# lambdaclass/ethrex

Measured on NVIDIA B200. Metric: bn254_g1_msm_points_per_sec, higher is better.
Workload: dtype u32x8 Montgomery (254-bit modular integer)

## Files before the change

### ethrex_b200/csrc/common.cuh

```cuda
#pragma once
#include <cuda_runtime.h>
#include <nvtx3/nvToolsExt.h>
#include <cstdint>
#include <cstdio>
#include <map>
#include <string>
#include <vector>

#include "../../include/b200zk.h"
#include "curve.cuh"
#include "bls381.cuh"

namespace b200zk {

template <> struct CurveB<Fp381> {
  static B2_D Fp381 b() { Fp381 four = Fp381::zero(); four.v[0] = 4; return Fp381::to_mont(four); }
};

struct DevBuf {
  void* p = nullptr;
  size_t cap = 0;
};

struct TwiddleSet {
  void* d = nullptr;
  size_t bytes = 0;
  uint32_t gen[8] = {0, 0, 0, 0, 0, 0, 0, 0};
  uint32_t root[8] = {0, 0, 0, 0, 0, 0, 0, 0};
  cudaEvent_t ready = nullptr;
};

struct SortSlot {
  DevBuf hist, offsets, cursor, run_off, tsum, digits, idx, key, ctab, cnt2;
  cudaEvent_t sorted = nullptr, released = nullptr;
};

struct BasesEntry {
  void* d = nullptr;
  size_t n = 0;
  bool g2 = false;
  bool bls = false;
  uint32_t table_c = 0;
};

}

struct b200zk_ctx {
  int device = 0;
  int sm_count = 148;
  cudaStream_t stream = nullptr;
  std::string last_error;
  uint64_t launches = 0;
  uint32_t msm_window = 0;
  uint32_t msm_chunks = 0;
  cudaStream_t stream_sort = nullptr;
  cudaEvent_t ev_in = nullptr;
  cudaEvent_t ev_up[64] = {};
  b200zk::SortSlot slot[2];
  b200zk::DevBuf ws_totals, ws_bitpart;
  b200zk::DevBuf ws_key, ws_ctab, ws_cnt2;
  b200zk::DevBuf ws_g16[4];
  b200zk::DevBuf ws_zinv;
  uint32_t zinv_log_n = 0xffffffffu;
  bool attr_sort = false, attr_acc = false, attr_ntt512 = false, attr_ntt256 = false;
  int msm_pair_rounds = -1;
  bool profiling = false;
  float phase_ms[6] = {0, 0, 0, 0, 0, 0};
  cudaEvent_t ev[8] = {};
  b200zk::DevBuf ws_hist, ws_offsets, ws_cursor, ws_blocksums, ws_idx, ws_buckets, ws_chunkS, ws_chunkV, ws_result,
      ws_points, ws_scalars, ws_ntt, ws_misc, ws_out, ws_segoff, ws_segbucket, ws_digits, ws_q0, ws_q1, ws_prefix, ws_info, ws_pairoff0, ws_pairoff1;
  uint32_t ntt_root[8] = {0x725b19f0u, 0x9bd61b6eu, 0x41112ed4u, 0x402d111eu, 0x8ef62abcu, 0x00e0a7ebu, 0xa58a7e85u, 0x2a3c09f0u};
  uint64_t ntt_root_id = 0;
  std::map<uint64_t, b200zk::TwiddleSet> twiddles;
  std::map<uint64_t, b200zk::BasesEntry> bases;
  uint64_t next_handle = 1;
  uint8_t* h_pinned = nullptr;
};

namespace b200zk {

inline int fail(b200zk_ctx* ctx, int status, const char* what, cudaError_t e = cudaSuccess) {
  if (ctx) {
    ctx->last_error = what;
    if (e != cudaSuccess) { ctx->last_error += ": "; ctx->last_error += cudaGetErrorString(e); }
  }
  return status;
}

#define B2_CUDA(ctx, expr)                                                      \
  do {                                                                          \
    cudaError_t _e = (expr);                                                    \
    if (_e != cudaSuccess) return b200zk::fail(ctx, _e == cudaErrorMemoryAllocation ? B200ZK_ERR_OOM : B200ZK_ERR_CUDA, #expr, _e); \
  } while (0)

#define B2_TRY(expr)                        \
  do {                                      \
    int _s = (expr);                        \
    if (_s > B200ZK_OK_INFINITY) return _s; \
  } while (0)

inline int ensure(b200zk_ctx* ctx, DevBuf& b, size_t bytes) {
  if (bytes <= b.cap) return B200ZK_OK;
  B2_CUDA(ctx, cudaDeviceSynchronize());
  if (b.p) { cudaFree(b.p); b.p = nullptr; b.cap = 0; }
  size_t want = bytes + bytes / 8;
  cudaError_t e = cudaMalloc(&b.p, want);
  if (e != cudaSuccess) { cudaGetLastError(); want = bytes; e = cudaMalloc(&b.p, want); }
  if (e != cudaSuccess) { cudaGetLastError(); b.p = nullptr; return fail(ctx, B200ZK_ERR_OOM, "cudaMalloc workspace", e); }
  b.cap = want;
  return B200ZK_OK;
}

struct DeviceGuard {
  int prev = -1;
  bool switched = false;
  explicit DeviceGuard(const b200zk_ctx* ctx) {
    if (!ctx) return;
    if (cudaGetDevice(&prev) != cudaSuccess) { cudaGetLastError(); prev = -1; }
    if (prev != ctx->device) { switched = cudaSetDevice(ctx->device) == cudaSuccess; if (!switched) cudaGetLastError(); }
  }
  ~DeviceGuard() { if (switched && prev >= 0) cudaSetDevice(prev); }
  DeviceGuard(const DeviceGuard&) = delete;
  DeviceGuard& operator=(const DeviceGuard&) = delete;
};

struct NvtxRange {
  explicit NvtxRange(const char* name) { nvtxRangePushA(name); }
  ~NvtxRange() { nvtxRangePop(); }
  NvtxRange(const NvtxRange&) = delete;
  NvtxRange& operator=(const NvtxRange&) = delete;
};

inline cudaStream_t pick_stream(b200zk_ctx* ctx, void* stream) { return stream ? (cudaStream_t)stream : ctx->stream; }

#define B2_LAUNCH(ctx, kernel, grid, block, smem, st, ...)                                   \
  do {                                                                                       \
    kernel<<<(grid), (block), (smem), (st)>>>(__VA_ARGS__);                                  \
    (ctx)->launches++;                                                                       \
    cudaError_t _e = cudaGetLastError();                                                     \
    if (_e != cudaSuccess) return b200zk::fail(ctx, B200ZK_ERR_CUDA, "launch " #kernel, _e); \
  } while (0)

template <class F> B2_D F load_fe(const void* base, size_t index) {
  const uint4* p = reinterpret_cast<const uint4*>(base) + 2 * index;
  uint4 lo = p[0], hi = p[1];
  F r;
  r.v[0] = lo.x; r.v[1] = lo.y; r.v[2] = lo.z; r.v[3] = lo.w;
// ... 91 lines not shown
```

### ethrex_b200/csrc/field.cuh

```cuda
#pragma once
#include <cstdint>

#define B2_HD __host__ __device__ __forceinline__
#define B2_D __device__ __forceinline__

namespace b200zk {

struct FqCfg {
  static B2_HD constexpr uint32_t mod(int i) {
    constexpr uint32_t m[8] = {0xd87cfd47u, 0x3c208c16u, 0x6871ca8du, 0x97816a91u, 0x8181585du, 0xb85045b6u, 0xe131a029u, 0x30644e72u};
    return m[i];
  }
  static B2_HD constexpr uint32_t r1(int i) {
    constexpr uint32_t m[8] = {0xc58f0d9du, 0xd35d438du, 0xf5c70b3du, 0x0a78eb28u, 0x7879462cu, 0x666ea36fu, 0x9a07df2fu, 0x0e0a77c1u};
    return m[i];
  }
  static B2_HD constexpr uint32_t r2(int i) {
    constexpr uint32_t m[8] = {0x538afa89u, 0xf32cfc5bu, 0xd44501fbu, 0xb5e71911u, 0x0a417ff6u, 0x47ab1effu, 0xcab8351fu, 0x06d89f71u};
    return m[i];
  }
  static constexpr uint32_t INV = 0xe4866389u;
};

struct FrCfg {
// ... 67 lines not shown
      : "r"(a2), "r"(a4), "r"(a6), "r"(b));
}
B2_D void mad_even_z2(uint32_t* x, uint32_t& top, uint32_t a4, uint32_t a6, uint32_t b) {
  asm("mad.lo.cc.u32  %0, %5, %7, %0;\n\t"
      "madc.hi.cc.u32 %1, %5, %7, %1;\n\t"
      "madc.lo.cc.u32 %2, %6, %7, %2;\n\t"
      "madc.hi.cc.u32 %3, %6, %7, %3;\n\t"
      "addc.u32       %4, %4, 0;"
      : "+r"(x[4]), "+r"(x[5]), "+r"(x[6]), "+r"(x[7]), "+r"(top)
      : "r"(a4), "r"(a6), "r"(b));
}
B2_D void mad_even_z3(uint32_t* x, uint32_t& top, uint32_t a6, uint32_t b) {
  asm("mad.lo.cc.u32  %0, %3, %4, %0;\n\t"
      "madc.hi.cc.u32 %1, %3, %4, %1;\n\t"
      "addc.u32       %2, %2, 0;"
      : "+r"(x[6]), "+r"(x[7]), "+r"(top)
      : "r"(a6), "r"(b));
}
B2_D void shift_mad_odd_z1(uint32_t* e, uint32_t& x0, uint32_t a3, uint32_t a5, uint32_t a7, uint32_t b) {
  asm("add.cc.u32     %8, %8, %1;\n\t"
      "addc.cc.u32    %0, %2, 0;\n\t"
      "addc.cc.u32    %1, %3, 0;\n\t"
      "madc.lo.cc.u32 %2, %9, %12, %4;\n\t"
      "madc.hi.cc.u32 %3, %9, %12, %5;\n\t"
      "madc.lo.cc.u32 %4, %10, %12, %6;\n\t"
      "madc.hi.cc.u32 %5, %10, %12, %7;\n\t"
      "madc.lo.cc.u32 %6, %11, %12, 0;\n\t"
      "madc.hi.u32    %7, %11, %12, 0;"
      : "+r"(e[0]), "+r"(e[1]), "+r"(e[2]), "+r"(e[3]), "+r"(e[4]), "+r"(e[5]), "+r"(e[6]), "+r"(e[7]), "+r"(x0)
      : "r"(a3), "r"(a5), "r"(a7), "r"(b));
}
B2_D void shift_mad_odd_z2(uint32_t* e, uint32_t& x0, uint32_t a5, uint32_t a7, uint32_t b) {
  asm("add.cc.u32     %8, %8, %1;\n\t"
      "addc.cc.u32    %0, %2, 0;\n\t"
      "addc.cc.u32    %1, %3, 0;\n\t"
      "addc.cc.u32    %2, %4, 0;\n\t"
      "addc.cc.u32    %3, %5, 0;\n\t"
      "madc.lo.cc.u32 %4, %9, %11, %6;\n\t"
      "madc.hi.cc.u32 %5, %9, %11, %7;\n\t"
      "madc.lo.cc.u32 %6, %10, %11, 0;\n\t"
      "madc.hi.u32    %7, %10, %11, 0;"
      : "+r"(e[0]), "+r"(e[1]), "+r"(e[2]), "+r"(e[3]), "+r"(e[4]), "+r"(e[5]), "+r"(e[6]), "+r"(e[7]), "+r"(x0)
      : "r"(a5), "r"(a7), "r"(b));
}
B2_D void shift_mad_odd_z3(uint32_t* e, uint32_t& x0, uint32_t a7, uint32_t b) {
  asm("add.cc.u32     %8, %8, %1;\n\t"
      "addc.cc.u32    %0, %2, 0;\n\t"
      "addc.cc.u32    %1, %3, 0;\n\t"
      "addc.cc.u32    %2, %4, 0;\n\t"
      "addc.cc.u32    %3, %5, 0;\n\t"
      "addc.cc.u32    %4, %6, 0;\n\t"
      "addc.cc.u32    %5, %7, 0;\n\t"
      "madc.lo.cc.u32 %6, %9, %10, 0;\n\t"
      "madc.hi.u32    %7, %9, %10, 0;"
      : "+r"(e[0]), "+r"(e[1]), "+r"(e[2]), "+r"(e[3]), "+r"(e[4]), "+r"(e[5]), "+r"(e[6]), "+r"(e[7]), "+r"(x0)
      : "r"(a7), "r"(b));
}

B2_D void mul_even(uint32_t* x, uint32_t a0, uint32_t a2, uint32_t a4, uint32_t a6, uint32_t b) {
  asm("mul.lo.u32 %0, %8,  %12;\n\t mul.hi.u32 %1, %8,  %12;\n\t"
      "mul.lo.u32 %2, %9,  %12;\n\t mul.hi.u32 %3, %9,  %12;\n\t"
      "mul.lo.u32 %4, %10, %12;\n\t mul.hi.u32 %5, %10, %12;\n\t"
      "mul.lo.u32 %6, %11, %12;\n\t mul.hi.u32 %7, %11, %12;"
      : "=r"(x[0]), "=r"(x[1]), "=r"(x[2]), "=r"(x[3]), "=r"(x[4]), "=r"(x[5]), "=r"(x[6]), "=r"(x[7])
      : "r"(a0), "r"(a2), "r"(a4), "r"(a6), "r"(b));
}

B2_D void add8(uint32_t* r, const uint32_t* a, const uint32_t* b) {
  asm("add.cc.u32  %0, %8,  %16;\n\t addc.cc.u32 %1, %9,  %17;\n\t addc.cc.u32 %2, %10, %18;\n\t addc.cc.u32 %3, %11, %19;\n\t"
      "addc.cc.u32 %4, %12, %20;\n\t addc.cc.u32 %5, %13, %21;\n\t addc.cc.u32 %6, %14, %22;\n\t addc.u32    %7, %15, %23;"
      : "=r"(r[0]), "=r"(r[1]), "=r"(r[2]), "=r"(r[3]), "=r"(r[4]), "=r"(r[5]), "=r"(r[6]), "=r"(r[7])
      : "r"(a[0]), "r"(a[1]), "r"(a[2]), "r"(a[3]), "r"(a[4]), "r"(a[5]), "r"(a[6]), "r"(a[7]),
        "r"(b[0]), "r"(b[1]), "r"(b[2]), "r"(b[3]), "r"(b[4]), "r"(b[5]), "r"(b[6]), "r"(b[7]));
}
B2_D uint32_t sub8(uint32_t* r, const uint32_t* a, const uint32_t* b) {
  uint32_t borrow;
  asm("sub.cc.u32  %0, %9,  %17;\n\t subc.cc.u32 %1, %10, %18;\n\t subc.cc.u32 %2, %11, %19;\n\t subc.cc.u32 %3, %12, %20;\n\t"
      "subc.cc.u32 %4, %13, %21;\n\t subc.cc.u32 %5, %14, %22;\n\t subc.cc.u32 %6, %15, %23;\n\t subc.cc.u32 %7, %16, %24;\n\t"
      "subc.u32    %8, 0, 0;"
      : "=r"(r[0]), "=r"(r[1]), "=r"(r[2]), "=r"(r[3]), "=r"(r[4]), "=r"(r[5]), "=r"(r[6]), "=r"(r[7]), "=r"(borrow)
      : "r"(a[0]), "r"(a[1]), "r"(a[2]), "r"(a[3]), "r"(a[4]), "r"(a[5]), "r"(a[6]), "r"(a[7]),
        "r"(b[0]), "r"(b[1]), "r"(b[2]), "r"(b[3]), "r"(b[4]), "r"(b[5]), "r"(b[6]), "r"(b[7]));
  return borrow;
}

}

template <class Cfg>
struct Fe {
  uint32_t v[8];

  static B2_HD Fe zero() { Fe r; for (int i = 0; i < 8; ++i) r.v[i] = 0; return r; }
  static B2_HD Fe one() { Fe r; for (int i = 0; i < 8; ++i) r.v[i] = Cfg::r1(i); return r; }
  static B2_HD Fe rsquared() { Fe r; for (int i = 0; i < 8; ++i) r.v[i] = Cfg::r2(i); return r; }
  static B2_HD Fe modulus() { Fe r; for (int i = 0; i < 8; ++i) r.v[i] = Cfg::mod(i); return r; }

  B2_HD bool is_zero() const {
    uint32_t o = 0;
#pragma unroll
    for (int i = 0; i < 8; ++i) o |= v[i];
    return o == 0;
  }
  B2_HD bool operator==(const Fe& b) const {
    uint32_t o = 0;
#pragma unroll
    for (int i = 0; i < 8; ++i) o |= v[i] ^ b.v[i];
    return o == 0;
  }
  B2_HD bool operator!=(const Fe& b) const { return !(*this == b); }

  static B2_D Fe reduce_once(const Fe& a) {
    Fe m = modulus(), t;
    uint32_t borrow = detail::sub8(t.v, a.v, m.v);
    Fe r;
#pragma unroll
    for (int i = 0; i < 8; ++i) r.v[i] = borrow ? a.v[i] : t.v[i];
    return r;
  }
  static B2_D Fe add(const Fe& a, const Fe& b) {
    Fe s; detail::add8(s.v, a.v, b.v);
    return reduce_once(s);
  }
  static B2_D Fe sub(const Fe& a, const Fe& b) {
    Fe d; uint32_t borrow = detail::sub8(d.v, a.v, b.v);
    Fe m;
#pragma unroll
    for (int i = 0; i < 8; ++i) m.v[i] = Cfg::mod(i) & borrow;
    Fe r; detail::add8(r.v, d.v, m.v);
    return r;
  }
  static B2_D Fe dbl(const Fe& a) { return add(a, a); }
  static B2_D Fe neg(const Fe& a) {
    Fe m = modulus(), r; detail::sub8(r.v, m.v, a.v);
    uint32_t nz = a.is_zero() ? 0u : 0xffffffffu;
#pragma unroll
    for (int i = 0; i < 8; ++i) r.v[i] &= nz;
    return r;
  }

  static B2_D Fe mul(const Fe& a, const Fe& b) {
    uint32_t ev[8], od[8];
    uint32_t m;
    detail::mul_even(ev, a.v[0], a.v[2], a.v[4], a.v[6], b.v[0]);
    detail::mul_even(od, a.v[1], a.v[3], a.v[5], a.v[7], b.v[0]);
    m = ev[0] * Cfg::INV;
    detail::mad_odd(od, Cfg::mod(1), Cfg::mod(3), Cfg::mod(5), Cfg::mod(7), m);
    detail::mad_even(ev, od[7], Cfg::mod(0), Cfg::mod(2), Cfg::mod(4), Cfg::mod(6), m);
#pragma unroll
    for (int i = 1; i < 8; i += 2) {
      detail::shift_mad_odd(ev, od[0], a.v[1], a.v[3], a.v[5], a.v[7], b.v[i]);
      detail::mad_even(od, ev[7], a.v[0], a.v[2], a.v[4], a.v[6], b.v[i]);
      m = od[0] * Cfg::INV;
      detail::mad_odd(ev, Cfg::mod(1), Cfg::mod(3), Cfg::mod(5), Cfg::mod(7), m);
      detail::mad_even(od, ev[7], Cfg::mod(0), Cfg::mod(2), Cfg::mod(4), Cfg::mod(6), m);
      if (i + 1 < 8) {
        detail::shift_mad_odd(od, ev[0], a.v[1], a.v[3], a.v[5], a.v[7], b.v[i + 1]);
        detail::mad_even(ev, od[7], a.v[0], a.v[2], a.v[4], a.v[6], b.v[i + 1]);
        m = ev[0] * Cfg::INV;
        detail::mad_odd(od, Cfg::mod(1), Cfg::mod(3), Cfg::mod(5), Cfg::mod(7), m);
        detail::mad_even(ev, od[7], Cfg::mod(0), Cfg::mod(2), Cfg::mod(4), Cfg::mod(6), m);
      }
    }
    Fe r;
    asm("add.cc.u32  %0, %8,  %16;\n\t addc.cc.u32 %1, %9,  %17;\n\t addc.cc.u32 %2, %10, %18;\n\t addc.cc.u32 %3, %11, %19;\n\t"
        "addc.cc.u32 %4, %12, %20;\n\t addc.cc.u32 %5, %13, %21;\n\t addc.cc.u32 %6, %14, %22;\n\t addc.u32    %7, %15, 0;"
        : "=r"(r.v[0]), "=r"(r.v[1]), "=r"(r.v[2]), "=r"(r.v[3]), "=r"(r.v[4]), "=r"(r.v[5]), "=r"(r.v[6]), "=r"(r.v[7])
// ... 80 lines not shown
        detail::mad_even(ev, od[7], c.v[0], c.v[2], c.v[4], c.v[6], d.v[i + 1]);
        m = ev[0] * Cfg::INV;
        detail::mad_odd(od, Cfg::mod(1), Cfg::mod(3), Cfg::mod(5), Cfg::mod(7), m);
        detail::mad_even(ev, od[7], Cfg::mod(0), Cfg::mod(2), Cfg::mod(4), Cfg::mod(6), m);
      }
    }
    Fe r;
    asm("add.cc.u32  %0, %8,  %16;\n\t addc.cc.u32 %1, %9,  %17;\n\t addc.cc.u32 %2, %10, %18;\n\t addc.cc.u32 %3, %11, %19;\n\t"
        "addc.cc.u32 %4, %12, %20;\n\t addc.cc.u32 %5, %13, %21;\n\t addc.cc.u32 %6, %14, %22;\n\t addc.u32    %7, %15, 0;"
        : "=r"(r.v[0]), "=r"(r.v[1]), "=r"(r.v[2]), "=r"(r.v[3]), "=r"(r.v[4]), "=r"(r.v[5]), "=r"(r.v[6]), "=r"(r.v[7])
        : "r"(ev[0]), "r"(ev[1]), "r"(ev[2]), "r"(ev[3]), "r"(ev[4]), "r"(ev[5]), "r"(ev[6]), "r"(ev[7]),
          "r"(od[1]), "r"(od[2]), "r"(od[3]), "r"(od[4]), "r"(od[5]), "r"(od[6]), "r"(od[7]));
    return reduce_once(r);
  }
  static B2_D Fe mul4_add(const Fe& a, const Fe& b, const Fe& c, const Fe& d, const Fe& e, const Fe& f, const Fe& g, const Fe& h) {
    const Fe* const x[4] = {&a, &c, &e, &g};
    const Fe* const y[4] = {&b, &d, &f, &h};
    uint32_t ev[8], od[8];
    uint32_t m;
    detail::mul_even(ev, a.v[0], a.v[2], a.v[4], a.v[6], b.v[0]);
    detail::mul_even(od, a.v[1], a.v[3], a.v[5], a.v[7], b.v[0]);
#pragma unroll
    for (int k = 1; k < 4; ++k) {
      detail::mad_odd(od, x[k]->v[1], x[k]->v[3], x[k]->v[5], x[k]->v[7], y[k]->v[0]);
      detail::mad_even(ev, od[7], x[k]->v[0], x[k]->v[2], x[k]->v[4], x[k]->v[6], y[k]->v[0]);
    }
    m = ev[0] * Cfg::INV;
    detail::mad_odd(od, Cfg::mod(1), Cfg::mod(3), Cfg::mod(5), Cfg::mod(7), m);
    detail::mad_even(ev, od[7], Cfg::mod(0), Cfg::mod(2), Cfg::mod(4), Cfg::mod(6), m);
#pragma unroll
    for (int i = 1; i < 8; i += 2) {
      detail::shift_mad_odd(ev, od[0], a.v[1], a.v[3], a.v[5], a.v[7], b.v[i]);
      detail::mad_even(od, ev[7], a.v[0], a.v[2], a.v[4], a.v[6], b.v[i]);
#pragma unroll
      for (int k = 1; k < 4; ++k) {
        detail::mad_odd(ev, x[k]->v[1], x[k]->v[3], x[k]->v[5], x[k]->v[7], y[k]->v[i]);
        detail::mad_even(od, ev[7], x[k]->v[0], x[k]->v[2], x[k]->v[4], x[k]->v[6], y[k]->v[i]);
      }
      m = od[0] * Cfg::INV;
      detail::mad_odd(ev, Cfg::mod(1), Cfg::mod(3), Cfg::mod(5), Cfg::mod(7), m);
      detail::mad_even(od, ev[7], Cfg::mod(0), Cfg::mod(2), Cfg::mod(4), Cfg::mod(6), m);
      if (i + 1 < 8) {
        detail::shift_mad_odd(od, ev[0], a.v[1], a.v[3], a.v[5], a.v[7], b.v[i + 1]);
        detail::mad_even(ev, od[7], a.v[0], a.v[2], a.v[4], a.v[6], b.v[i + 1]);
#pragma unroll
        for (int k = 1; k < 4; ++k) {
          detail::mad_odd(od, x[k]->v[1], x[k]->v[3], x[k]->v[5], x[k]->v[7], y[k]->v[i + 1]);
          detail::mad_even(ev, od[7], x[k]->v[0], x[k]->v[2], x[k]->v[4], x[k]->v[6], y[k]->v[i + 1]);
        }
        m = ev[0] * Cfg::INV;
        detail::mad_odd(od, Cfg::mod(1), Cfg::mod(3), Cfg::mod(5), Cfg::mod(7), m);
        detail::mad_even(ev, od[7], Cfg::mod(0), Cfg::mod(2), Cfg::mod(4), Cfg::mod(6), m);
      }
    }
    Fe r;
    asm("add.cc.u32  %0, %8,  %16;\n\t addc.cc.u32 %1, %9,  %17;\n\t addc.cc.u32 %2, %10, %18;\n\t addc.cc.u32 %3, %11, %19;\n\t"
        "addc.cc.u32 %4, %12, %20;\n\t addc.cc.u32 %5, %13, %21;\n\t addc.cc.u32 %6, %14, %22;\n\t addc.u32    %7, %15, 0;"
        : "=r"(r.v[0]), "=r"(r.v[1]), "=r"(r.v[2]), "=r"(r.v[3]), "=r"(r.v[4]), "=r"(r.v[5]), "=r"(r.v[6]), "=r"(r.v[7])
        : "r"(ev[0]), "r"(ev[1]), "r"(ev[2]), "r"(ev[3]), "r"(ev[4]), "r"(ev[5]), "r"(ev[6]), "r"(ev[7]),
          "r"(od[1]), "r"(od[2]), "r"(od[3]), "r"(od[4]), "r"(od[5]), "r"(od[6]), "r"(od[7]));
    return reduce_once(r);
  }
  static B2_D Fe mul2_sub(const Fe& a, const Fe& b, const Fe& c, const Fe& d) { return mul2_add(a, b, neg(c), d); }

  static B2_D Fe to_mont(const Fe& canonical) { return mul(canonical, rsquared()); }
  static B2_D Fe from_mont(const Fe& a) {
    Fe o = zero(); o.v[0] = 1; return mul(a, o);
  }
  static B2_D Fe pow(const Fe& a, const uint32_t* e) {
    Fe acc = one();
    for (int i = 255; i >= 0; --i) {
      acc = sqr(acc);
      if ((e[i >> 5] >> (i & 31)) & 1) acc = mul(acc, a);
    }
    return acc;
  }
  static B2_D Fe inv(const Fe& a) {
    uint32_t e[8];
#pragma unroll
    for (int i = 0; i < 8; ++i) e[i] = Cfg::mod(i);
    e[0] -= 2;
    return pow(a, e);
  }
};

typedef Fe<FqCfg> Fq;
typedef Fe<FrCfg> Fr;

struct Fq2 {
  Fq c0, c1;
  static B2_D Fq2 zero() { return {Fq::zero(), Fq::zero()}; }
  static B2_D Fq2 one() { return {Fq::one(), Fq::zero()}; }
  B2_D bool is_zero() const { return c0.is_zero() && c1.is_zero(); }
  B2_D bool operator==(const Fq2& b) const { return c0 == b.c0 && c1 == b.c1; }
  B2_D bool operator!=(const Fq2& b) const { return !(*this == b); }
  static B2_D Fq2 add(const Fq2& a, const Fq2& b) { return {Fq::add(a.c0, b.c0), Fq::add(a.c1, b.c1)}; }
  static B2_D Fq2 sub(const Fq2& a, const Fq2& b) { return {Fq::sub(a.c0, b.c0), Fq::sub(a.c1, b.c1)}; }
  static B2_D Fq2 dbl(const Fq2& a) { return {Fq::dbl(a.c0), Fq::dbl(a.c1)}; }
  static B2_D Fq2 neg(const Fq2& a) { return {Fq::neg(a.c0), Fq::neg(a.c1)}; }
  static B2_D Fq2 mul(const Fq2& a, const Fq2& b) {
    return {Fq::mul2_add(a.c0, b.c0, Fq::neg(a.c1), b.c1), Fq::mul2_add(a.c0, b.c1, a.c1, b.c0)};
  }
  static B2_D Fq2 sqr(const Fq2& a) {
    Fq s = Fq::add(a.c0, a.c1), d = Fq::sub(a.c0, a.c1), m = Fq::mul(a.c0, a.c1);
    return {Fq::mul(s, d), Fq::dbl(m)};
  }
  static B2_D Fq2 mul2_sub(const Fq2& a, const Fq2& b, const Fq2& c, const Fq2& d) {
#ifdef B200ZK_FQ2_NO_MUL4
    return sub(mul(a, b), mul(c, d));
#else
    const Fq na1 = Fq::neg(a.c1), nc0 = Fq::neg(c.c0), nc1 = Fq::neg(c.c1);
    return {Fq::mul4_add(a.c0, b.c0, na1, b.c1, nc0, d.c0, c.c1, d.c1), Fq::mul4_add(a.c0, b.c1, a.c1, b.c0, nc0, d.c1, nc1, d.c0)};
#endif
  }
  static B2_D Fq2 inv(const Fq2& a) {
    Fq d = Fq::inv(Fq::add(Fq::sqr(a.c0), Fq::sqr(a.c1)));
    return {Fq::mul(a.c0, d), Fq::neg(Fq::mul(a.c1, d))};
  }
};

}
```

### ethrex_b200/csrc/msm.cu

```cuda
#include "common.cuh"
#include "tma.cuh"
#include <cstdlib>

namespace b200zk {

static constexpr int kMaxWindows = 64;
static constexpr uint32_t kMaxPipelineChunks = 64;
static constexpr int kChunk = 16;
static constexpr int kG2MinBlocks = 1;

struct MsmPlan {
  uint32_t c, W, B;
  uint32_t chunk, T;
  uint32_t merged;
  uint32_t Wr;
  uint32_t table_stride;
  uint32_t adaptive;
};

uint32_t precompute_window(size_t n) {
  uint32_t lg = 0;
  while (((size_t)1 << lg) < n) ++lg;
  if (lg >= 20) return 20;
  if (lg <= 6) return 6;
// ... 493 lines not shown
  for (int k = 0; k < kScanItems; ++k) { v[k] = base + k < G ? scan_value(in, aux, base + k, seg, shift) : 0; s += v[k]; }
  uint32_t incl = s;
#pragma unroll
  for (int o = 1; o < 32; o <<= 1) { uint32_t t = __shfl_up_sync(0xffffffffu, incl, o); if ((threadIdx.x & 31) >= (unsigned)o) incl += t; }
  if ((threadIdx.x & 31) == 31) warp_tot[threadIdx.x >> 5] = incl;
  __syncthreads();
  uint32_t wbase = 0;
  for (unsigned k = 0; k < (threadIdx.x >> 5); ++k) wbase += warp_tot[k];
  uint32_t run = tile_offsets[blockIdx.x] + wbase + incl - s;
#pragma unroll
  for (int k = 0; k < kScanItems; ++k) {
    if (base + k < G) { offsets[base + k] = seg ? run + (aux[base + k] + seg - 1) / seg : run; if (cursor) cursor[base + k] = run; }
    run += v[k];
  }
  if (blockIdx.x == gridDim.x - 1 && threadIdx.x == kScanThreads - 1) offsets[G] = seg ? run + (aux[G] + seg - 1) / seg : run;
}

static constexpr uint32_t kSegLenMax = 256;
static constexpr uint32_t kTreeRadix = 64;
static constexpr uint32_t kDirectRuns = 4;

static uint32_t pick_slice_len(size_t M, size_t resident) {
  if (M == 0) return kSegLenMax;
  size_t per_thread = (M + resident - 1) / resident;
  size_t waves = (per_thread + kSegLenMax - 1) / kSegLenMax;
  size_t len = (M + resident * waves - 1) / (resident * waves);
  if (len < 16) len = 16;
  if (len > kSegLenMax) len = kSegLenMax;
  return (uint32_t)len;
}

B2_D uint32_t bucket_of(const uint32_t* __restrict__ offsets, uint32_t G, uint32_t lo, uint32_t e) {
  uint32_t step = 1, hi = lo + 1;
  while (hi < G && __ldg(offsets + hi) <= e) { lo = hi; step <<= 1; hi = lo + step; }
  if (hi > G) hi = G;
  while (hi - lo > 1) {
    uint32_t mid = (lo + hi) >> 1;
    if (__ldg(offsets + mid) <= e) lo = mid; else hi = mid;
  }
  return lo;
}

template <class F, bool DIRECT, int MINB = 1>
__global__ void __launch_bounds__(128, MINB) msm_accumulate(const void* __restrict__ points, const uint32_t* __restrict__ idx,
                                                      const uint32_t* __restrict__ offsets, const uint32_t* __restrict__ run_off,
                                                      uint32_t G, uint32_t kSegLen, void* __restrict__ partials, uint32_t* __restrict__ run_bucket) {
  const uint32_t t = blockIdx.x * blockDim.x + threadIdx.x;
  const uint32_t M = __ldg(offsets + G);
  const uint64_t e0_64 = (uint64_t)t * kSegLen;
  if (e0_64 >= M) return;
  const uint32_t e0 = (uint32_t)e0_64;
  const uint32_t e1 = (M - e0 > kSegLen) ? e0 + kSegLen : M;
  uint32_t g;
  {
    uint32_t lo = 0, hi = G;
    while (hi - lo > 1) { uint32_t mid = (lo + hi) >> 1; if (__ldg(offsets + mid) <= e0) lo = mid; else hi = mid; }
    g = lo;
  }
  const uint32_t off0 = __ldg(offsets + g);
  uint32_t slot = t + (__ldg(run_off + g) - (off0 + kSegLen - 1) / kSegLen) + ((off0 % kSegLen) ? 1u : 0u);
  uint32_t next = __ldg(offsets + g + 1);
  XYZZ<F> acc = XYZZ<F>::identity();
  uint32_t v = DIRECT ? e0 : __ldg(idx + e0);
  Affine<F> p = load_affine_nc<F>(points, v & 0x7fffffffu);
  for (uint32_t e = e0; e < e1; ++e) {
    uint32_t vn = v; Affine<F> pn = p;
    if (e + 1 < e1) { vn = DIRECT ? e + 1 : __ldg(idx + e + 1); pn = load_affine_nc<F>(points, vn & 0x7fffffffu); }
    if (e == next) {
      store_xyzz(partials, slot, acc);
      run_bucket[slot] = g;
      ++slot;
      acc = XYZZ<F>::identity();
      g = bucket_of(offsets, G, g + 1, e);
      next = __ldg(offsets + g + 1);
    }
    if (!DIRECT && (v >> 31)) p.y = F::neg(p.y);
    xyzz_add_mixed(acc, p.x, p.y);
    v = vn; p = pn;
  }
  store_xyzz(partials, slot, acc);
  run_bucket[slot] = g;
}

__device__ __noinline__ Fq fq_mul_call(Fq a, Fq b) { return Fq::mul(a, b); }
__device__ __noinline__ Fq fq_mul2_add_call(Fq a, Fq b, Fq c, Fq d) { return Fq::mul2_add(a, b, c, d); }
__device__ __noinline__ Fq fq_mul4_add_call(Fq a, Fq b, Fq c, Fq d, Fq e, Fq f, Fq g, Fq h) { return Fq::mul4_add(a, b, c, d, e, f, g, h); }

struct PairLane {
  uint32_t mask;
  bool hi;
  B2_D Fq partner(const Fq& a) const {
    Fq r;
#pragma unroll
    for (int i = 0; i < 8; ++i) r.v[i] = __shfl_xor_sync(mask, a.v[i], 1);
    return r;
  }
  B2_D bool both(bool mine) const { return __shfl_xor_sync(mask, mine ? 1u : 0u, 1) != 0 && mine; }
  B2_D Fq sel(const Fq& if_hi, const Fq& if_lo) const {
    Fq r;
#pragma unroll
    for (int i = 0; i < 8; ++i) r.v[i] = hi ? if_hi.v[i] : if_lo.v[i];
    return r;
  }
  B2_D Fq mul(const Fq& a, const Fq& pa, const Fq& b, const Fq& pb) const {
    return fq_mul2_add_call(a, sel(pb, b), sel(pa, Fq::neg(pa)), sel(b, pb));
  }
  B2_D Fq sqr(const Fq& a, const Fq& pa) const {
    return fq_mul_call(sel(Fq::dbl(a), Fq::add(a, pa)), sel(pa, Fq::sub(a, pa)));
  }
  B2_D Fq mul2_sub(const Fq& a, const Fq& pa, const Fq& b, const Fq& pb, const Fq& c, const Fq& pc, const Fq& d, const Fq& pd) const {
    const Fq nc = Fq::neg(c);
    return fq_mul4_add_call(sel(pa, a), b, sel(a, Fq::neg(pa)), pb, sel(Fq::neg(pc), nc), d, sel(nc, pc), pd);
  }
  B2_D Fq one() const { return hi ? Fq::zero() : Fq::one(); }
};
struct XYZZHalf { Fq x, y, zz, zzz; };

B2_D void pair_mdbl(const PairLane& L, XYZZHalf& acc, const Fq& x1, const Fq& y1) {
  const Fq U = Fq::dbl(y1), pU = L.partner(U);
  const Fq V = L.sqr(U, pU), pV = L.partner(V);
  const Fq W = L.mul(U, pU, V, pV), pW = L.partner(W);
  const Fq px1 = L.partner(x1), py1 = L.partner(y1);
  const Fq S = L.mul(x1, px1, V, pV);
  const Fq xx = L.sqr(x1, px1), M = Fq::add(Fq::dbl(xx), xx), pM = L.partner(M);
  acc.x = Fq::sub(L.sqr(M, pM), Fq::dbl(S));
  const Fq T = Fq::sub(S, acc.x), pT = L.partner(T);
  acc.y = L.mul2_sub(M, pM, T, pT, W, pW, y1, py1);
  acc.zz = V; acc.zzz = W;
}
B2_D void pair_add_mixed(const PairLane& L, XYZZHalf& acc, const Fq& x2, const Fq& y2) {
  if (L.both(x2.is_zero() && y2.is_zero())) return;
  if (L.both(acc.zz.is_zero())) { acc.x = x2; acc.y = y2; acc.zz = L.one(); acc.zzz = L.one(); return; }
  const Fq pzz = L.partner(acc.zz), pzzz = L.partner(acc.zzz);
  const Fq U2 = L.mul(x2, L.partner(x2), acc.zz, pzz), S2 = L.mul(y2, L.partner(y2), acc.zzz, pzzz);
  const Fq P = Fq::sub(U2, acc.x), R = Fq::sub(S2, acc.y);
  if (L.both(P.is_zero())) {
    if (L.both(R.is_zero())) pair_mdbl(L, acc, x2, y2);
    else { acc.x = Fq::zero(); acc.y = Fq::zero(); acc.zz = Fq::zero(); acc.zzz = Fq::zero(); }
    return;
  }
  const Fq pP = L.partner(P);
  const Fq PP = L.sqr(P, pP), pPP = L.partner(PP);
  const Fq PPP = L.mul(P, pP, PP, pPP), pPPP = L.partner(PPP);
  const Fq Q = L.mul(acc.x, L.partner(acc.x), PP, pPP);
  const Fq pR = L.partner(R);
  const Fq x3 = Fq::sub(Fq::sub(L.sqr(R, pR), PPP), Fq::dbl(Q));
  const Fq T = Fq::sub(Q, x3), pT = L.partner(T);
  acc.y = L.mul2_sub(R, pR, T, pT, acc.y, L.partner(acc.y), PPP, pPPP);
  acc.x = x3;
  acc.zz = L.mul(acc.zz, pzz, PP, pPP);
  acc.zzz = L.mul(acc.zzz, pzzz, PPP, pPPP);
}

template <int MINB>
__global__ void __launch_bounds__(128, MINB) msm_accumulate_g2_pair(const void* __restrict__ points, const uint32_t* __restrict__ idx, const uint32_t* __restrict__ offsets,
                                                                const uint32_t* __restrict__ run_off, uint32_t G, uint32_t kSegLen, void* __restrict__ partials,
                                                                uint32_t* __restrict__ run_bucket) {
  const uint32_t gt = blockIdx.x * blockDim.x + threadIdx.x;
  const uint32_t t = gt >> 1;
  PairLane L;
  L.hi = (threadIdx.x & 1) != 0;
  L.mask = 3u << (threadIdx.x & 30);
  const uint32_t M = __ldg(offsets + G);
  const uint64_t e0_64 = (uint64_t)t * kSegLen;
  if (e0_64 >= M) return;
  const uint32_t e0 = (uint32_t)e0_64;
// ... 305 lines not shown
}
template <class F> __global__ void write_identity(void* result) {
  if (blockIdx.x || threadIdx.x) return;
  store_xyzz(result, 0, XYZZ<F>::identity());
}

B2_D void store_be32(uint8_t* out, const Fq& canonical) {
  uint32_t* o = reinterpret_cast<uint32_t*>(out);
#pragma unroll
  for (int k = 0; k < 8; ++k) o[k] = __byte_perm(canonical.v[7 - k], 0, 0x0123);
}
B2_D void encode_point(uint8_t* out, const Affine<Fq>& p, bool native) {
  if (native) { store_affine<Fq>(out, 0, p); return; }
  store_be32(out, Fq::from_mont(p.x)); store_be32(out + 32, Fq::from_mont(p.y));
}
B2_D void encode_point(uint8_t* out, const Affine<Fq2>& p, bool native) {
  if (native) { store_affine<Fq2>(out, 0, p); return; }
  store_be32(out, Fq::from_mont(p.x.c1)); store_be32(out + 32, Fq::from_mont(p.x.c0));
  store_be32(out + 64, Fq::from_mont(p.y.c1)); store_be32(out + 96, Fq::from_mont(p.y.c0));
}
B2_D void encode_point(uint8_t* out, const Affine<Fp381>& p, bool native) {
  if (native) { store_affine<Fp381>(out, 0, p); return; }
  uint32_t* o = reinterpret_cast<uint32_t*>(out);
#pragma unroll
  for (int k = 0; k < 24; ++k) o[k] = 0;
  if (p.is_inf()) { out[0] = 0xc0; return; }
  const Fp381 x = Fp381::from_mont(p.x), y = Fp381::from_mont(p.y);
  Fp381 half;
#pragma unroll
  for (int i = 0; i < 12; ++i) half.v[i] = Fp381Cfg::half(i);
#pragma unroll
  for (int k = 0; k < 12; ++k) o[k] = __byte_perm(x.v[11 - k], 0, 0x0123);
  out[0] |= 0x80 | (Fp381::less(half, y) ? 0x20 : 0x00);
}
template <class F>
__global__ void msm_encode(const void* __restrict__ partials, size_t count, bool native, uint8_t* __restrict__ out) {
  if (blockIdx.x || threadIdx.x) return;
  XYZZ<F> acc = XYZZ<F>::identity();
  for (size_t k = 0; k < count; ++k) { XYZZ<F> p = load_xyzz<F>(partials, k); xyzz_add(acc, p); }
  Affine<F> a = xyzz_to_affine(acc);
  encode_point(out, a, native);
  *reinterpret_cast<uint32_t*>(out + 2 * FieldBytes<F>::value) = a.is_inf() ? 1u : 0u;
}

__global__ void groth16_assemble(const uint8_t* __restrict__ partials, size_t count, uint8_t* __restrict__ out) {
  if (threadIdx.x) return;
  const uint32_t which = blockIdx.x;
  uint32_t* inf = reinterpret_cast<uint32_t*>(out + 320);
  if (which == 1) {
    XYZZ<Fq2> acc = XYZZ<Fq2>::identity();
    for (size_t k = 0; k < count; ++k) { XYZZ<Fq2> p = load_xyzz<Fq2>(partials + k * 768 + 256, 0); xyzz_add(acc, p); }
    Affine<Fq2> a = xyzz_to_affine(acc);
    encode_point(out + 64, a, false);
    inf[1] = a.is_inf() ? 1u : 0u;
    return;
  }
  XYZZ<Fq> acc = XYZZ<Fq>::identity();
  const size_t off = which == 0 ? 0 : (which == 3 ? 128 : 512);
  for (size_t k = 0; k < count; ++k) {
    XYZZ<Fq> p = load_xyzz<Fq>(partials + k * 768 + off, 0);
    xyzz_add(acc, p);
    if (which == 2) { XYZZ<Fq> h = load_xyzz<Fq>(partials + k * 768 + 640, 0); xyzz_add(acc, h); }
  }
  Affine<Fq> a = xyzz_to_affine(acc);
  encode_point(out + (which == 0 ? 0 : (which == 2 ? 192 : 256)), a, false);
  inf[which == 0 ? 0 : (which == 2 ? 2 : 3)] = a.is_inf() ? 1u : 0u;
}
int groth16_assemble_dev(b200zk_ctx* ctx, const void* d_partials, size_t count, cudaStream_t st, void* d_out) {
  B2_LAUNCH(ctx, groth16_assemble, 4, 32, 0, st, (const uint8_t*)d_partials, count, (uint8_t*)d_out);
  return B200ZK_OK;
}

static inline void phase_mark(b200zk_ctx* ctx, int k, cudaStream_t st) {
  if (ctx->profiling) cudaEventRecord(ctx->ev[k], st);
}

static int g2_pair_knob() {
  static int k = -1;
  if (k < 0) { const char* e = getenv("B200ZK_G2_PAIR"); k = (e && (*e == '0' || *e == '3' || *e == '4')) ? (*e - '0') : 3; }
  return k;
}
template <class F> static size_t resident_slices(const b200zk_ctx* ctx) {
  if (IsFq2<F>::value) { const int k = g2_pair_knob(); return (size_t)ctx->sm_count * (k ? 64u * (unsigned)k : 256u); }
  return (size_t)ctx->sm_count * (sizeof(F) > 32 ? 256u : 512u);
}
template <class F>
static int launch_accumulate(b200zk_ctx* ctx, cudaStream_t st, const void* pts, const uint32_t* idx, const uint32_t* offsets, const uint32_t* run_off, uint32_t G, uint32_t L,
                             size_t slices, void* partials, uint32_t* run_bucket) {
  const unsigned agrid = (unsigned)((slices + 127) / 128);
  if constexpr (IsFq2<F>::value) {
    const int k = g2_pair_knob();
    const unsigned pgrid = (unsigned)((2 * slices + 127) / 128);
    if (k == 3) B2_LAUNCH(ctx, msm_accumulate_g2_pair<3>, pgrid, 128, 0, st, pts, idx, offsets, run_off, G, L, partials, run_bucket);
    else if (k == 4) B2_LAUNCH(ctx, msm_accumulate_g2_pair<4>, pgrid, 128, 0, st, pts, idx, offsets, run_off, G, L, partials, run_bucket);
    else B2_LAUNCH(ctx, (msm_accumulate<F, false, 1>), agrid, 128, 0, st, pts, idx, offsets, run_off, G, L, partials, run_bucket);
  } else {
    B2_LAUNCH(ctx, (msm_accumulate<F, false>), agrid, 128, 0, st, pts, idx, offsets, run_off, G, L, partials, run_bucket);
  }
  return B200ZK_OK;
}

static int legacy_sort_knob() {
  static int knob = -1;
  if (knob < 0) { const char* e = getenv("B200ZK_SORT"); knob = (e && !strcmp(e, "legacy")) ? 1 : 0; }
  return knob;
}
static double chunk_ratio_knob(double dflt) {
  const char* e = getenv("B200ZK_CHUNK_RATIO");
  double r = (e && *e) ? atof(e) : dflt;
  return (r >= 1.0 && r <= 64.0) ? r : dflt;
}
static size_t sort_ctab_bytes(int sm_count) { return (2 * ((size_t)kSortMaxBins * (size_t)sm_count + 1) + kSortMaxBins + 1) * 4; }
static size_t sort_cnt2_bytes(size_t M_max) { return (M_max / kFineSeg + kSortMaxBins + 1) * (size_t)kSortMaxFine * 4; }
static int run_two_level_sort(b200zk_ctx* ctx, const void* d_scalars, size_t n, uint32_t flags, const MsmPlan& pl, const SortPlan& sp, uint32_t* hist, uint32_t* offsets,
                              uint32_t* tsum, uint2* ent1, uint32_t* ctab, uint32_t* cnt2, uint32_t* idx, cudaStream_t st, bool mark) {
  const size_t Gc = (size_t)sp.C * sp.NC, tilesC = (Gc + kScanTile - 1) / kScanTile;
  const size_t G = sp.G, tilesG = (G + kScanTile - 1) / kScanTile;
  uint32_t *cnt = ctab, *base = ctab + Gc + 1, *item_start = base + Gc + 1;
  if (!ctx->attr_sort) {
    B2_CUDA(ctx, cudaFuncSetAttribute(msm_sort_coarse, cudaFuncAttributeMaxDynamicSharedMemorySize, (int)sizeof(SortCoarseSmem)));
    B2_CUDA(ctx, cudaFuncSetAttribute(msm_sort_fine_place, cudaFuncAttributeMaxDynamicSharedMemorySize, (int)sizeof(SortFineSmem)));
    ctx->attr_sort = true;
  }
  B2_CUDA(ctx, cudaMemsetAsync(cnt, 0, (Gc + 1) * 4, st));
  B2_LAUNCH(ctx, msm_sort_count, sp.NC * kSortCountSub, kHistTile, 0, st, d_scalars, n, flags, pl, sp, cnt);
  if (mark) phase_mark(ctx, 1, st);
  B2_LAUNCH(ctx, scan_tile_sums, (unsigned)tilesC, kScanThreads, 0, st, (const uint32_t*)cnt, (const uint32_t*)nullptr, Gc, 0u, 0u, tsum);
  B2_LAUNCH(ctx, scan_tile_offsets, 1, 1024, 0, st, tsum, tilesC);
  B2_LAUNCH(ctx, scan_apply, (unsigned)tilesC, kScanThreads, 0, st, (const uint32_t*)cnt, (const uint32_t*)nullptr, Gc, 0u, 0u, (const uint32_t*)tsum, base, (uint32_t*)nullptr);
  if (mark) phase_mark(ctx, 2, st);
  B2_LAUNCH(ctx, msm_sort_coarse, sp.NC, kSortTile, sizeof(SortCoarseSmem), st, d_scalars, n, flags, pl, sp, (const uint32_t*)base, ent1);
  const unsigned max_items = (unsigned)((n * (size_t)pl.W) / kFineSeg + sp.C + 1);
  const uint32_t F = 1u << sp.fb;
  B2_LAUNCH(ctx, msm_sort_items, 1, 1024, 0, st, (const uint32_t*)base, sp, item_start);
  B2_LAUNCH(ctx, msm_sort_fine_count, max_items, 1024, 0, st, (const uint2*)ent1, sp, (const uint32_t*)base, (const uint32_t*)item_start, cnt2);
  B2_LAUNCH(ctx, msm_sort_fine_prefix, (unsigned)(((size_t)sp.C * F + 255) / 256), 256, 0, st, sp, (const uint32_t*)item_start, cnt2, hist);
  B2_LAUNCH(ctx, scan_tile_sums, (unsigned)tilesG, kScanThreads, 0, st, (const uint32_t*)hist, (const uint32_t*)nullptr, G, 0u, 0u, tsum);
  B2_LAUNCH(ctx, scan_tile_offsets, 1, 1024, 0, st, tsum, tilesG);
  B2_LAUNCH(ctx, scan_apply, (unsigned)tilesG, kScanThreads, 0, st, (const uint32_t*)hist, (const uint32_t*)nullptr, G, 0u, 0u, (const uint32_t*)tsum, offsets, (uint32_t*)nullptr);
  B2_LAUNCH(ctx, msm_sort_fine_place, max_items, 1024, sizeof(SortFineSmem), st, (const uint2*)ent1, sp, (const uint32_t*)base, (const uint32_t*)item_start, (const uint32_t*)cnt2,
            (const uint32_t*)offsets, idx);
  return B200ZK_OK;
}

template <class F>
static int msm_run_pipelined(b200zk_ctx* ctx, const void* d_points, const void* d_scalars, const void* h_scalars, size_t n, uint32_t flags,
                             cudaStream_t st, void* d_partial, const MsmPlan& pl, uint32_t K) {
  const size_t G = (size_t)pl.Wr * pl.B;
  const size_t tiles = (G + kScanTile - 1) / kScanTile;
  const size_t xy = 4 * FieldBytes<F>::value, pt = 2 * FieldBytes<F>::value;
  size_t bnd[kMaxPipelineChunks + 1];
  uint32_t chunks = 0;
  {
    const double r = h_scalars ? chunk_ratio_knob(IsFq2<F>::value ? 12.0 : 4.0) : 1.0;
    double tot = 0, w = 1;
    for (uint32_t k = 0; k < K; ++k) { tot += w; w *= r; }
    double cum = 0; w = 1;
    bnd[0] = 0;
    for (uint32_t k = 0; k < K; ++k) {
      cum += w; w *= r;
      size_t hi = (k == K - 1) ? n : std::min(n, (((size_t)((double)n * (cum / tot))) + 1023) & ~(size_t)1023);
      if (hi > bnd[chunks]) bnd[++chunks] = hi;
    }
  }
  size_t chunk = 0;
  for (uint32_t k = 0; k < chunks; ++k) chunk = std::max(chunk, bnd[k + 1] - bnd[k]);
  const size_t Mk_max = chunk * pl.W;
  const size_t resident = resident_slices<F>(ctx);
  uint32_t Lk[kMaxPipelineChunks];
  size_t S_max = 0;
  for (uint32_t k = 0; k < chunks; ++k) {
    const size_t Mk = (bnd[k + 1] - bnd[k]) * pl.W;
    Lk[k] = pick_slice_len(Mk, resident);
    S_max = std::max(S_max, Mk / Lk[k] + 1 + G);
  }
  SortPlan sp0;
  const bool two_level = !legacy_sort_knob() && make_sort_plan(chunk, pl, ctx->sm_count, &sp0);
  const size_t Gc = (size_t)kSortMaxBins * (size_t)ctx->sm_count;
  for (int sl = 0; sl < 2; ++sl) {
    SortSlot& s = ctx->slot[sl];
// ... 286 lines not shown
```

Before: 469.0 million.

## Accumulate BN254 G1 buckets in affine form with batched safegcd inversion

Replaces the XYZZ bucket accumulation kernel for G1 with an affine-coordinate kernel. Each thread handles J=8 segments, batches their slope denominators with Montgomery's trick, and inverts the product with a new constant-time Bernstein-Yang divstep inversion. Chain state lives in shared memory. The aim is fewer field multiplications per point addition, paid for by extra shared memory, lower occupancy, per-step inversion latency, branch divergence on the special cases, and a changed slice count.

```diff
diff --git a/ethrex_b200/csrc/common.cuh b/ethrex_b200/csrc/common.cuh
--- a/ethrex_b200/csrc/common.cuh
+++ b/ethrex_b200/csrc/common.cuh
@@ -62,7 +62,7 @@
   b200zk::DevBuf ws_g16[4];
   b200zk::DevBuf ws_zinv;
   uint32_t zinv_log_n = 0xffffffffu;
-  bool attr_sort = false, attr_acc = false, attr_ntt512 = false, attr_ntt256 = false;
+  bool attr_sort = false, attr_acc = false, attr_ntt512 = false, attr_ntt256 = false, attr_affine = false;
   int msm_pair_rounds = -1;
   bool profiling = false;
   float phase_ms[6] = {0, 0, 0, 0, 0, 0};
diff --git a/ethrex_b200/csrc/field.cuh b/ethrex_b200/csrc/field.cuh
--- a/ethrex_b200/csrc/field.cuh
+++ b/ethrex_b200/csrc/field.cuh
@@ -173,6 +173,56 @@
       : "r"(a[0]), "r"(a[1]), "r"(a[2]), "r"(a[3]), "r"(a[4]), "r"(a[5]), "r"(a[6]), "r"(a[7]),
         "r"(b[0]), "r"(b[1]), "r"(b[2]), "r"(b[3]), "r"(b[4]), "r"(b[5]), "r"(b[6]), "r"(b[7]));
   return borrow;
+}
+
+B2_D uint32_t sign_mask(uint32_t w) { return (uint32_t)((int32_t)w >> 31); }
+
+B2_D int32_t divsteps_30(int32_t zeta, uint32_t f, uint32_t g, uint32_t& u_, uint32_t& v_, uint32_t& q_, uint32_t& r_) {
+  uint32_t u = 1, v = 0, q = 0, r = 1;
+#pragma unroll
+  for (int i = 0; i < 30; ++i) {
+    uint32_t c1 = (uint32_t)(zeta >> 31);
+    const uint32_t c2 = 0u - (g & 1u);
+    const uint32_t x = (f ^ c1) - c1, y = (u ^ c1) - c1, z = (v ^ c1) - c1;
+    g += x & c2; q += y & c2; r += z & c2;
+    c1 &= c2;
+    zeta = (int32_t)(((uint32_t)zeta ^ c1) - 1u);
+    f += g & c1; u += q & c1; v += r & c1;
+    g >>= 1; u <<= 1; v <<= 1;
+  }
+  u_ = u; v_ = v; q_ = q; r_ = r;
+  return zeta;
+}
+B2_D void mul_word9(uint32_t* t, const uint32_t* a, uint32_t w) {
+  uint64_t c = 0;
+#pragma unroll
+  for (int i = 0; i < 8; ++i) { c = (uint64_t)a[i] * w + (c >> 32); t[i] = (uint32_t)c; }
+  t[8] = (uint32_t)(c >> 32);
+}
+B2_D void lin9(uint32_t* t, const uint32_t* a, const uint32_t* b, uint32_t u, uint32_t v) {
+  uint32_t ta[9], tb[9];
+  mul_word9(ta, a, u);
+  mul_word9(tb, b, v);
+  const uint32_t su = sign_mask(u), sv = sign_mask(v);
+  uint64_t c = (uint64_t)ta[0] + tb[0];
+  t[0] = (uint32_t)c;
+  int64_t s = (int64_t)(c >> 32);
+#pragma unroll
+  for (int i = 1; i < 9; ++i) {
+    s += (int64_t)ta[i] + tb[i] - (int64_t)(a[i - 1] & su) - (int64_t)(b[i - 1] & sv);
+    t[i] = (uint32_t)s;
+    s >>= 32;
+  }
+}
+B2_D void shr30(uint32_t* r, const uint32_t* t) {
+#pragma unroll
+  for (int i = 0; i < 8; ++i) r[i] = __funnelshift_r(t[i], t[i + 1], 30);
+}
+B2_D void lin_fg(uint32_t* r, const uint32_t* a, const uint32_t* b, uint32_t u, uint32_t v) {
+  uint32_t t[9];
+  lin9(t, a, b, u, v);
+  t[8] -= (u & sign_mask(a[7])) + (v & sign_mask(b[7]));
+  shr30(r, t);
 }
 
 }
@@ -419,6 +469,49 @@
     e[0] -= 2;
     return pow(a, e);
   }
+
+  static B2_D Fe lin_mod(const Fe& a, const Fe& b, uint32_t u, uint32_t v) {
+    uint32_t t[9], kp[9];
+    detail::lin9(t, a.v, b.v, u, v);
+    const uint32_t k = (t[0] * Cfg::INV) & 0x3fffffffu;
+    const Fe m = modulus();
+    detail::mul_word9(kp, m.v, k);
+    uint64_t c = 0;
+#pragma unroll
+    for (int i = 0; i < 9; ++i) { c = (uint64_t)t[i] + kp[i] + (c >> 32); t[i] = (uint32_t)c; }
+    Fe r, mm;
+    detail::shr30(r.v, t);
+    const uint32_t s = detail::sign_mask(r.v[7]);
+#pragma unroll
+    for (int i = 0; i < 8; ++i) mm.v[i] = m.v[i] & s;
+    detail::add8(r.v, r.v, mm.v);
+    return reduce_once(r);
+  }
+  static B2_D Fe inv_gcd(const Fe& a) {
+    uint32_t f[8], g[8];
+    Fe d = zero(), e = rsquared();
+#pragma unroll
+    for (int i = 0; i < 8; ++i) { f[i] = Cfg::mod(i); g[i] = a.v[i]; }
+    int32_t zeta = -1;
+#pragma unroll 1
+    for (int rnd = 0; rnd < 20; ++rnd) {
+      uint32_t u, v, q, r;
+      zeta = detail::divsteps_30(zeta, f[0], g[0], u, v, q, r);
+      uint32_t nf[8], ng[8];
+      detail::lin_fg(nf, f, g, u, v);
+      detail::lin_fg(ng, f, g, q, r);
+#pragma unroll
+      for (int i = 0; i < 8; ++i) { f[i] = nf[i]; g[i] = ng[i]; }
+      const Fe nd = lin_mod(d, e, u, v);
+      e = lin_mod(d, e, q, r);
+      d = nd;
+      uint32_t gz = 0;
+#pragma unroll
+      for (int i = 0; i < 8; ++i) gz |= g[i];
+      if (__all_sync(__activemask(), gz == 0)) break;
+    }
+    return (f[7] >> 31) ? neg(d) : d;
+  }
 };
 
 typedef Fe<FqCfg> Fq;
diff --git a/ethrex_b200/csrc/msm.cu b/ethrex_b200/csrc/msm.cu
--- a/ethrex_b200/csrc/msm.cu
+++ b/ethrex_b200/csrc/msm.cu
@@ -599,6 +599,129 @@
   run_bucket[slot] = g;
 }
 
+static constexpr int kAffJ = 8;
+static constexpr int kAffThreads = 128;
+static constexpr int kAffMinBlocks = 2;
+struct AffChainState { uint32_t g, next, slot; };
+template <int J>
+struct AffSmem {
+  uint4 f[3][J][2][kAffThreads];
+  uint32_t st[3][J][kAffThreads];
+};
+
+template <int J>
+__global__ void __launch_bounds__(kAffThreads, kAffMinBlocks) msm_accumulate_affine(const void* __restrict__ points, const uint32_t* __restrict__ idx,
+                                                                                 const uint32_t* __restrict__ offsets, const uint32_t* __restrict__ run_off,
+                                                                                 uint32_t G, uint32_t kSegLen, void* __restrict__ partials,
+                                                                                 uint32_t* __restrict__ run_bucket) {
+  extern __shared__ __align__(16) uint8_t smem_raw[];
+  AffSmem<J>& sm = *reinterpret_cast<AffSmem<J>*>(smem_raw);
+  const uint32_t tid = threadIdx.x;
+  const uint32_t t = blockIdx.x * blockDim.x + tid;
+  const uint32_t M = __ldg(offsets + G);
+  const uint64_t first_e = (uint64_t)t * J * kSegLen;
+  if (first_e >= M) return;
+  auto ld = [&](int fld, int j) -> Fq {
+    const uint4 a = sm.f[fld][j][0][tid], b = sm.f[fld][j][1][tid];
+    Fq r; r.v[0] = a.x; r.v[1] = a.y; r.v[2] = a.z; r.v[3] = a.w; r.v[4] = b.x; r.v[5] = b.y; r.v[6] = b.z; r.v[7] = b.w;
+    return r;
+  };
+  auto st = [&](int fld, int j, const Fq& r) {
+    sm.f[fld][j][0][tid] = make_uint4(r.v[0], r.v[1], r.v[2], r.v[3]);
+    sm.f[fld][j][1][tid] = make_uint4(r.v[4], r.v[5], r.v[6], r.v[7]);
+  };
+  auto e0_of = [&](int j) -> uint32_t { const uint64_t e = ((uint64_t)t * J + j) * kSegLen; return e < M ? (uint32_t)e : M; };
+  auto e1_of = [&](int j) -> uint32_t { const uint32_t e = e0_of(j); return (M - e > kSegLen) ? e + kSegLen : M; };
+#pragma unroll 1
+  for (int j = 0; j < J; ++j) {
+    const uint32_t e0 = e0_of(j);
+    uint32_t g = 0, slot = 0, next = 0;
+    if (e0 < M) {
+      uint32_t lo = 0, hi = G;
+      while (hi - lo > 1) { uint32_t mid = (lo + hi) >> 1; if (__ldg(offsets + mid) <= e0) lo = mid; else hi = mid; }
+      g = lo;
+      const uint32_t off0 = __ldg(offsets + g);
+      slot = (t * J + j) + (__ldg(run_off + g) - (off0 + kSegLen - 1) / kSegLen) + ((off0 % kSegLen) ? 1u : 0u);
+      next = __ldg(offsets + g + 1);
+    }
+    sm.st[0][j][tid] = g; sm.st[1][j][tid] = next; sm.st[2][j][tid] = slot;
+    st(0, j, Fq::zero()); st(1, j, Fq::zero());
+  }
+  auto gather = [&](int j, uint32_t s) -> Affine<Fq> {
+    const uint32_t e = e0_of(j) + s;
+    if (e >= e1_of(j)) return {Fq::zero(), Fq::zero()};
+    const uint32_t v = __ldg(idx + e);
+    Affine<Fq> p = load_affine_nc<Fq>(points, v & 0x7fffffffu);
+    if (v >> 31) p.y = Fq::neg(p.y);
+    return p;
+  };
+  auto denom = [&](const Affine<Fq>& a, const Affine<Fq>& p, int* kind) -> Fq {
+    if (p.is_inf()) { *kind = 3; return Fq::one(); }
+    if (a.is_inf()) { *kind = 2; return Fq::one(); }
+    const Fq dx = Fq::sub(p.x, a.x);
+    if (!dx.is_zero()) { *kind = 0; return dx; }
+    if (p.y == a.y) { *kind = 1; return Fq::dbl(a.y); }
+    *kind = 4; return Fq::one();
+  };
+#pragma unroll 1
+  for (uint32_t s = 0; s < kSegLen; ++s) {
+    Fq prod = Fq::one();
+    Affine<Fq> pn = gather(0, s);
+#pragma unroll 1
+    for (int j = 0; j < J; ++j) {
+      const Affine<Fq> p = pn;
+      if (j + 1 < J) pn = gather(j + 1, s);
+      const uint32_t e = e0_of(j) + s;
+      Affine<Fq> a = {ld(0, j), ld(1, j)};
+      if (e < e1_of(j) && e == sm.st[1][j][tid]) {
+        const uint32_t slot = sm.st[2][j][tid];
+        store_xyzz(partials, slot, xyzz_from_affine(a));
+        run_bucket[slot] = sm.st[0][j][tid];
+        const uint32_t g = bucket_of(offsets, G, sm.st[0][j][tid] + 1, e);
+        sm.st[0][j][tid] = g; sm.st[1][j][tid] = __ldg(offsets + g + 1); sm.st[2][j][tid] = slot + 1;
+        a = {Fq::zero(), Fq::zero()};
+        st(0, j, a.x); st(1, j, a.y);
+      }
+      int kind;
+      const Fq d = denom(a, p, &kind);
+      st(2, j, prod);
+      prod = j == 0 ? d : Fq::mul(prod, d);
+    }
+    Fq inv = Fq::inv_gcd(prod);
+    pn = gather(J - 1, s);
+#pragma unroll 1
+    for (int j = J - 1; j >= 0; --j) {
+      const Affine<Fq> p = pn;
+      if (j > 0) pn = gather(j - 1, s);
+      const Affine<Fq> a = {ld(0, j), ld(1, j)};
+      int kind;
+      const Fq d = denom(a, p, &kind);
+      Fq dinv = inv;
+      if (j > 0) { dinv = Fq::mul(inv, ld(2, j)); inv = Fq::mul(inv, d); }
+      if (kind <= 1) {
+        Fq num;
+        if (kind == 0) num = Fq::sub(p.y, a.y);
+        else { const Fq xx = Fq::sqr(a.x); num = Fq::add(Fq::dbl(xx), xx); }
+        const Fq lam = Fq::mul(num, dinv);
+        const Fq x3 = Fq::sub(Fq::sub(Fq::sqr(lam), a.x), p.x);
+        const Fq y3 = Fq::sub(Fq::mul(lam, Fq::sub(a.x, x3)), a.y);
+        st(0, j, x3); st(1, j, y3);
+      } else if (kind == 2) {
+        st(0, j, p.x); st(1, j, p.y);
+      } else if (kind == 4) {
+        st(0, j, Fq::zero()); st(1, j, Fq::zero());
+      }
+    }
+  }
+#pragma unroll 1
+  for (int j = 0; j < J; ++j) {
+    if (e0_of(j) >= M) continue;
+    const uint32_t slot = sm.st[2][j][tid];
+    store_xyzz(partials, slot, xyzz_from_affine(Affine<Fq>{ld(0, j), ld(1, j)}));
+    run_bucket[slot] = sm.st[0][j][tid];
+  }
+}
+
 __device__ __noinline__ Fq fq_mul_call(Fq a, Fq b) { return Fq::mul(a, b); }
 __device__ __noinline__ Fq fq_mul2_add_call(Fq a, Fq b, Fq c, Fq d) { return Fq::mul2_add(a, b, c, d); }
 __device__ __noinline__ Fq fq_mul4_add_call(Fq a, Fq b, Fq c, Fq d, Fq e, Fq f, Fq g, Fq h) { return Fq::mul4_add(a, b, c, d, e, f, g, h); }
@@ -1070,7 +1193,8 @@
 }
 template <class F> static size_t resident_slices(const b200zk_ctx* ctx) {
   if (IsFq2<F>::value) { const int k = g2_pair_knob(); return (size_t)ctx->sm_count * (k ? 64u * (unsigned)k : 256u); }
-  return (size_t)ctx->sm_count * (sizeof(F) > 32 ? 256u : 512u);
+  if (sizeof(F) > 32) return (size_t)ctx->sm_count * 256u;
+  return (size_t)ctx->sm_count * (kAffThreads * kAffMinBlocks * kAffJ);
 }
 template <class F>
 static int launch_accumulate(b200zk_ctx* ctx, cudaStream_t st, const void* pts, const uint32_t* idx, const uint32_t* offsets, const uint32_t* run_off, uint32_t G, uint32_t L,
@@ -1082,8 +1206,16 @@
     if (k == 3) B2_LAUNCH(ctx, msm_accumulate_g2_pair<3>, pgrid, 128, 0, st, pts, idx, offsets, run_off, G, L, partials, run_bucket);
     else if (k == 4) B2_LAUNCH(ctx, msm_accumulate_g2_pair<4>, pgrid, 128, 0, st, pts, idx, offsets, run_off, G, L, partials, run_bucket);
     else B2_LAUNCH(ctx, (msm_accumulate<F, false, 1>), agrid, 128, 0, st, pts, idx, offsets, run_off, G, L, partials, run_bucket);
+  } else if constexpr (sizeof(F) > 32) {
+    B2_LAUNCH(ctx, (msm_accumulate<F, false>), agrid, 128, 0, st, pts, idx, offsets, run_off, G, L, partials, run_bucket);
   } else {
-    B2_LAUNCH(ctx, (msm_accumulate<F, false>), agrid, 128, 0, st, pts, idx, offsets, run_off, G, L, partials, run_bucket);
+    const size_t threads = (slices + kAffJ - 1) / kAffJ;
+    const unsigned fgrid = (unsigned)((threads + kAffThreads - 1) / kAffThreads);
+    if (!ctx->attr_affine) {
+      B2_CUDA(ctx, cudaFuncSetAttribute(msm_accumulate_affine<kAffJ>, cudaFuncAttributeMaxDynamicSharedMemorySize, (int)sizeof(AffSmem<kAffJ>)));
+      ctx->attr_affine = true;
+    }
+    B2_LAUNCH(ctx, msm_accumulate_affine<kAffJ>, fgrid, kAffThreads, sizeof(AffSmem<kAffJ>), st, pts, idx, offsets, run_off, G, L, partials, run_bucket);
   }
   return B200ZK_OK;
 }
```

After: 181.8 million, median of 6. -61.2%, worse.
